# lmdu/pyfastx

Hardware: AMD Instinct MI355X
Metric: FASTA index build + 1M random 100bp subseq fetches, 3 Gbp plain FASTA per GPU (throughput of the whole step, stream resident in HBM) (higher is better)
Workload: dtype u8; 1 GPU; configs[1]: synthetic 3.0 Gbp hg38-shaped plain FASTA per GPU (200 contigs, 60-col LF, soft-masked, N runs), index build + 1000000 random 100 bp intervals (50% '-' strand); parallelism=one GPU, the whole stream resident in its HBM

## Files before the change

pyfastx_amd/csrc/fx_kernels.hpp:

```cpp
#pragma once
#include <hip/hip_runtime.h>
#include <stdint.h>

namespace fx {

constexpr int BLOCK = 256;
constexpr int UNROLL = 8;
constexpr int CHUNK = 16;
constexpr int TILE = BLOCK * CHUNK * UNROLL;

__device__ __forceinline__ uint32_t zero_bytes(uint32_t x) {
    return ~(((x & 0x7F7F7F7Fu) + 0x7F7F7F7Fu) | x | 0x7F7F7F7Fu);
}
__device__ __forceinline__ uint32_t flags4(uint32_t t) { return __builtin_amdgcn_udot4(t, 0x08040201u, 0u, false) >> 7; }
__device__ __forceinline__ uint32_t eq_mask16(const uint4 &v, uint32_t pat) {
    uint32_t lo = __builtin_amdgcn_udot4(zero_bytes(v.x ^ pat), 0x08040201u, 0u, false);
    lo = __builtin_amdgcn_udot4(zero_bytes(v.y ^ pat), 0x80402010u, lo, false);
    uint32_t hi = __builtin_amdgcn_udot4(zero_bytes(v.z ^ pat), 0x08040201u, 0u, false);
    hi = __builtin_amdgcn_udot4(zero_bytes(v.w ^ pat), 0x80402010u, hi, false);
    return (lo >> 7) | (hi << 1);
}

__device__ __forceinline__ uint4 load16(const uint8_t *__restrict__ data, int64_t p, int64_t n) {
    if (p + CHUNK <= n) return *reinterpret_cast<const uint4 *>(data + p);
// ... 327 lines not shown
                    uint32_t word = w[0];
#pragma unroll
                    for (int k = 1; k < NW; ++k) word = (j >> 2) == k ? w[k] : word;
                    uint8_t c = (uint8_t)(word >> ((j & 3) * 8));
                    if ((fl & 1) && c >= 'a' && c <= 'z') c -= 32;
                    if (fl & 4) c = lut[c];
                    const int64_t o = r - skip;
                    out[(fl & 2) ? (take - 1 - o) : o] = c;
                }
                ++r;
            }
            rank += total;
        }
        if (ok) {
            int64_t got = rank - skip;
            got = got < 0 ? 0 : (got > take ? take : got);
            if ((fl & 2) && got < take && got > 0) {
                const int64_t delta = take - got;
                for (int64_t j0 = 0; j0 < got; j0 += G) {
                    const int64_t j = j0 + sub;
                    uint8_t c = 0;
                    if (j < got) c = out[delta + j];
                    if (j < got) out[j] = c;
                }
            }
            if (sub == 0 && q.out_len) q.out_len[i] = got;
        }
    }
}

template <int G, int NP, bool COAL = false>
__global__ __launch_bounds__(BLOCK) void k_fetch_lines(const uint8_t *__restrict__ data, int64_t gbase, int64_t n_bytes, FetchQ q, FastaTab tab,
                                                      int64_t nq, int flags_all, uint8_t *__restrict__ dst, int32_t *__restrict__ list,
                                                      int *__restrict__ list_n) {
    __shared__ uint8_t lut[256];
    constexpr int CO_CAP = 2048;
    __shared__ __attribute__((aligned(16))) uint32_t s_out[COAL ? BLOCK / 64 : 1][COAL ? (CO_CAP + 32) / 4 : 1];
    constexpr int TABCAP = 512;
    __shared__ int64_t s_boff[TABCAP], s_slen[TABCAP];
    __shared__ int32_t s_llen[TABCAP], s_en[TABCAP];
    const int64_t n_seq = tab.n_seq_dev ? (*tab.n_seq_dev < tab.n_seq ? (int64_t)*tab.n_seq_dev : tab.n_seq) : tab.n_seq;
    const bool tab_lds = n_seq <= TABCAP && n_seq > 0;
    build_comp_lut(lut);
    if (tab_lds)
        for (int r = threadIdx.x; r < (int)n_seq; r += BLOCK) {
            s_boff[r] = tab.boff[r]; s_slen[r] = tab.slen[r];
            const int64_t ll = tab.llen[r];
            s_llen[r] = ll > 0x7FFFFFFFll ? 0x7FFFFFFF : (int32_t)ll;
            s_en[r] = tab.elen[r] | (tab.norm[r] << 8);
        }
    __syncthreads();
    constexpr int QPW = 64 / G;
    const int lane = lane_id(), sub = lane & (G - 1), grp = lane / G;
    const int64_t wave = ((int64_t)blockIdx.x * BLOCK + threadIdx.x) >> 6;
    const int64_t nwaves = ((int64_t)gridDim.x * BLOCK) >> 6;
    int64_t d_id = 0, d_a = 0, d_b = 0, d_off = 0;
    int d_fl = flags_all;
    auto fetch_desc = [&](int64_t i) {
        if (i >= nq) return;
        d_id = q.seq_id[i]; d_a = q.start[i]; d_b = q.stop[i];
        d_off = q.dst_off[i];
        d_fl = q.qflags ? q.qflags[i] : flags_all;
    };
    fetch_desc(wave * QPW + grp);
    for (int64_t i0 = wave * QPW; i0 < nq; i0 += nwaves * QPW) {
        const int64_t i = i0 + grp;
        const bool live = i < nq;
        const int64_t id = d_id, a = d_a, b = d_b;
// ... 339 lines not shown
```

pyfastx_amd/csrc/fx_spanscan.hpp:

```cpp
#pragma once
#include "fx_kernels.hpp"

namespace fx {

#ifndef FX_GRAN
#define FX_GRAN 4096
#endif
constexpr int GRAN = FX_GRAN;
constexpr int GR_ROWS = GRAN / (64 * CHUNK);
constexpr int SPAN_GRANS = 65536 / GRAN;
constexpr int SPAN = GRAN * SPAN_GRANS;
constexpr uint32_t SP_NONE = 0xFFFFFFFFu;

struct GranOut { uint32_t n, h, first, last, v1, c1, v2, c2, ovf; };
struct __attribute__((aligned(16))) GranPk { uint32_t nh, fl, d1, d2; };
__device__ __forceinline__ GranPk gran_pack(const GranOut &o) {
    GranPk p;
    p.nh = o.n | (o.h << 16); p.fl = (o.first & 0xFFFFu) | (o.last << 16);
    p.d1 = o.v1 | (o.c1 << 16); p.d2 = o.v2 | (o.c2 << 16) | (o.ovf << 31);
    return p;
}
__device__ __forceinline__ GranOut gran_unpack(const GranPk &p) {
    GranOut o;
    o.n = p.nh & 0xFFFFu; o.h = p.nh >> 16;
// ... 240 lines not shown
    const int lo = __shfl((int)(v & 0xFFFFFFFFll), l, 64), hi = __shfl((int)(v >> 32), l, 64);
    return ((long long)hi << 32) | (unsigned int)lo;
}
struct Tri { long long n, h, last; };
__device__ __forceinline__ Tri tri_join(const Tri &a, const Tri &b) { return Tri{a.n + b.n, a.h + b.h, a.last > b.last ? a.last : b.last}; }
__device__ __forceinline__ Tri tri_wave_incl(Tri v) {
    const int l = lane_id();
#pragma unroll
    for (int d = 1; d < 64; d <<= 1) {
        const Tri t{shfl_up64(v.n, d), shfl_up64(v.h, d), shfl_up64(v.last, d)};
        if (l >= d) v = tri_join(t, v);
    }
    return v;
}
__device__ __forceinline__ Tri tri_block_incl(Tri v, Tri *lds, Tri *total) {
    const int w = threadIdx.x >> 6, l = lane_id(), nw = (blockDim.x + 63) >> 6;
    const Tri inc = tri_wave_incl(v);
    __syncthreads();
    if (l == 63) lds[w] = inc;
    __syncthreads();
    Tri base{0, 0, -1}, tot{0, 0, -1};
    for (int i = 0; i < nw; ++i) { const Tri s = lds[i]; if (i < w) base = tri_join(base, s); tot = tri_join(tot, s); }
    *total = tot;
    return tri_join(base, inc);
}
__device__ __forceinline__ Tri gran_tri(const GranPk *__restrict__ go, int64_t g, int64_t ngran, int64_t gbase) {
    if (g >= ngran) return Tri{0, 0, -1};
    const GranOut o = gran_unpack(go[g]);
    return Tri{(long long)o.n, (long long)o.h, o.n ? gbase + g * (long long)GRAN + o.last : -1};
}

template <int MODE, int CG>
__global__ __launch_bounds__(CG) void k_gran_reduce(const uint8_t *__restrict__ data, int64_t n, int prev_byte,
                                                   int is_last, GranList hgl, GranPk *__restrict__ go,
                                                   int64_t ngran, int64_t gbase, ChunkTot *__restrict__ ct) {
    __shared__ Tri lds[CG / 64];
    if (blockIdx.x == gridDim.x - 1) {
        if (threadIdx.x < 64) {
            uint32_t L = 0;
            const uint32_t h_w = granule<false, MODE>(data, n, prev_byte, is_last, ngran - 1, go, L);
            if (MODE == 0 && h_w && threadIdx.x == 0) hgl.g[atomicAdd(hgl.count, 1u)] = (uint32_t)(ngran - 1);
        }
        __threadfence_block();
        __syncthreads();
    }
    Tri tot;
    tri_block_incl(gran_tri(go, (int64_t)blockIdx.x * CG + threadIdx.x, ngran, gbase), lds, &tot);
    if (threadIdx.x == 0) ct[blockIdx.x] = ChunkTot{tot.n, tot.h, tot.last, 0};
}

struct Tri32 { uint32_t n, h; int32_t last; };
__device__ __forceinline__ Tri32 tri32_block_incl(Tri32 v, uint32_t (*lds)[16], Tri32 *total) {
    const int w = threadIdx.x >> 6, l = lane_id(), nw = (blockDim.x + 63) >> 6;
#pragma unroll
    for (int d = 1; d < 64; d <<= 1) {
        const uint32_t a = __shfl_up(v.n, d, 64), b = __shfl_up(v.h, d, 64);
        const int32_t c = __shfl_up(v.last, d, 64);
        if (l >= d) { v.n += a; v.h += b; v.last = c > v.last ? c : v.last; }
    }
    __syncthreads();
    if (l == 63) { lds[0][w] = v.n; lds[1][w] = v.h; lds[2][w] = (uint32_t)v.last; }
    __syncthreads();
    Tri32 base{0, 0, -1}, tot{0, 0, -1};
    for (int i = 0; i < nw; ++i) {
        const uint32_t a = lds[0][i], b = lds[1][i];
        const int32_t c = (int32_t)lds[2][i];
        if (i < w) { base.n += a; base.h += b; base.last = c > base.last ? c : base.last; }
        tot.n += a; tot.h += b; tot.last = c > tot.last ? c : tot.last;
    }
    *total = tot;
    return Tri32{base.n + v.n, base.h + v.h, base.last > v.last ? base.last : v.last};
}

template <int CG>
__global__ __launch_bounds__(CG) void k_gran_prefix(const GranPk *__restrict__ go, int64_t ngran, int64_t gbase,
                                                            const ChunkTot *__restrict__ ct, Totals *__restrict__ tot,
                                                            int64_t *__restrict__ nl_prefix, int64_t *__restrict__ hdr_prefix,
                                                            int64_t *__restrict__ prevnl) {
    __shared__ Tri lds[CG / 64];
    __shared__ uint32_t lds32[3][16];
    Tri b{0, 0, -1};
    for (int64_t c = threadIdx.x; c < (int64_t)blockIdx.x; c += CG) { const ChunkTot t = ct[c]; b = tri_join(b, Tri{t.n, t.h, t.last}); }
    Tri base{0, 0, -1};
    if (blockIdx.x) tri_block_incl(b, lds, &base);
    const int64_t g = (int64_t)blockIdx.x * CG + threadIdx.x;
    Tri32 v{0, 0, -1};
    if (g < ngran) {
        const GranOut o = gran_unpack(go[g]);
        v = Tri32{o.n, o.h, o.n ? (int32_t)(threadIdx.x * GRAN + o.last) : -1};
    }
    Tri32 total;
    const Tri32 inc = tri32_block_incl(v, lds32, &total);
    const int64_t cstart = gbase + (int64_t)blockIdx.x * CG * GRAN;
    if (g < ngran) {
        nl_prefix[g] = base.n + (inc.n - v.n);
        hdr_prefix[g] = base.h + (inc.h - v.h);
        int32_t pm = __shfl_up(inc.last, 1, 64);
        if (lane_id() == 0) { pm = -1; for (int i = 0; i < (int)(threadIdx.x >> 6); ++i) { const int32_t c = (int32_t)lds32[2][i]; pm = c > pm ? c : pm; } }
        prevnl[g] = pm >= 0 ? cstart + pm : base.last;
    }
    if (blockIdx.x == gridDim.x - 1 && threadIdx.x == 0) {
        const int64_t tn = base.n + total.n, th = base.h + total.h, tl = total.last >= 0 ? cstart + total.last : base.last;
        nl_prefix[ngran] = tn; hdr_prefix[ngran] = th; prevnl[ngran] = tl;
        tot->n_nl = tn; tot->n_hdr = th; tot->last_nl = tl;
    }
}

struct ScanCtx {
    const uint8_t *data; int64_t n, gbase, ngran;
    const GranPk *go;
    const int64_t *nl_prefix, *hdr_prefix, *prevnl;
};

__device__ __forceinline__ int64_t next_nl(const ScanCtx &c, int64_t x) {
    const int64_t y = x + 1 - c.gbase;
    if (y > c.n) return -1;
    const int64_t g = y / GRAN;
    if (g < c.ngran) {
        const GranOut o = gran_unpack(c.go[g]);
        const int64_t gs = g * (int64_t)GRAN;
        if (o.n && gs + o.last >= y) {
            if (gs + o.first >= y) return c.gbase + gs + o.first;
            for (int64_t p = y & ~(int64_t)(CHUNK - 1); p < gs + GRAN; p += CHUNK) {
                const uint4 v = load16(c.data, p, c.n);
                uint32_t m = eq_mask16(v, 0x0A0A0A0Au);
                if (p < y) m &= 0xFFFFu << (y - p);
                if (m) return c.gbase + p + (__ffs(m) - 1);
                if (p + CHUNK > c.n) break;
            }
            return c.gbase + gs + o.last;
        }
    }
    const int64_t key = c.gbase + (g + 1) * (int64_t)GRAN;
    int64_t lo = g + 1, hi = c.ngran;
    if (lo >= hi || c.prevnl[c.ngran] < key) return -1;
    while (lo < hi) { const int64_t mid = (lo + hi) >> 1; if (c.prevnl[mid + 1] >= key) hi = mid; else lo = mid + 1; }
    return c.gbase + lo * (int64_t)GRAN + (c.go[lo].fl & 0xFFFFu);
// ... 281 lines not shown
            if (mism) atomicAdd(&rv.bad[r], mism);
            return;
        }
    }
    irr.g[atomicAdd(irr.count, 1u)] = (uint32_t)g;
}

__global__ __launch_bounds__(BLOCK) void k_gran_exact(ScanCtx x, RecView rv, int64_t cap, GranList irr, int is_last, int prev_byte) {
    const int lane = lane_id();
    const int64_t wave = ((int64_t)blockIdx.x * blockDim.x + threadIdx.x) >> 6;
    const int64_t nwaves = ((int64_t)gridDim.x * blockDim.x) >> 6;
    const int64_t cnt = *irr.count;
    int64_t i = wave, g = i < cnt ? irr.g[i] : 0;
    uint4 v[GR_ROWS];
    if (i < cnt) {
#pragma unroll
        for (int j = 0; j < GR_ROWS; ++j) v[j] = load16(x.data, g * (int64_t)GRAN + j * 1024 + lane * CHUNK, x.n);
    }
    for (; i < cnt; i += nwaves) {
        const int64_t gc = g, hb = x.hdr_prefix[gc];
        int64_t he = x.hdr_prefix[gc + 1];
        if (he > cap) he = cap;
        ExactMasks mk;
        exact_masks(x, v, is_last, prev_byte, gc, he > hb, mk);
        if (i + nwaves < cnt) {
            g = irr.g[i + nwaves];
#pragma unroll
            for (int j = 0; j < GR_ROWS; ++j) v[j] = load16(x.data, g * (int64_t)GRAN + j * 1024 + lane * CHUNK, x.n);
        }
        exact_rows(x, rv, cap, gc, hb, mk);
    }
}

__global__ __launch_bounds__(BLOCK) void k_fasta_finalize2(int64_t cap, FastaCols c, Totals *__restrict__ tot,
                                                          const uint8_t *__restrict__ data, int64_t n_bytes, int64_t gbase) {
    const int64_t *__restrict__ hdr = c.hoff, *__restrict__ hdr_line = c.hdr_line;
    const int64_t k = (int64_t)blockIdx.x * BLOCK + threadIdx.x;
    const int64_t n_hdr = tot->n_hdr < cap ? tot->n_hdr : cap;
    int64_t s = 0;
    if (k < n_hdr) {
        if (c.dlen[k] >= 0) {
            int64_t hn, Ln;
            if (k + 1 < n_hdr) { hn = hdr[k + 1]; Ln = hdr_line[k + 1]; }
            else               { hn = tot->last_nl + 1; Ln = tot->n_nl; }
            const int64_t nseq = Ln - hdr_line[k] - 1;
            const int64_t blen = hn - c.boff[k];
            s = blen - (int64_t)c.elen[k] * nseq;
            c.blen[k] = blen; c.slen[k] = s;
            const int norm = c.bad[k] > 1 ? 0 : 1;
            c.norm[k] = norm;
            int reg = line_regular(data, n_bytes, gbase, c.boff[k], blen, s, nseq > 0 ? c.llen[k] : 0, c.elen[k], norm);
            if (reg < 0) reg = c.bad[k] == 0;
            c.reg[k] = reg;
        } else { c.blen[k] = 0; c.slen[k] = 0; c.norm[k] = 1; c.reg[k] = 0; }
    }
    __shared__ unsigned long long blk;
    if (threadIdx.x == 0) blk = 0;
    __syncthreads();
    s = wave_sum64(s);
    if (lane_id() == 0 && s) atomicAdd(&blk, (unsigned long long)s);
    __syncthreads();
    if (threadIdx.x == 0 && blk) atomicAdd((unsigned long long *)&tot->seq_len, blk);
}

__global__ __launch_bounds__(BLOCK) void k_line_regular(const uint8_t *__restrict__ data, int64_t n_bytes, int64_t gbase, int64_t n,
                                                       const int64_t *__restrict__ boff, const int64_t *__restrict__ blen,
                                                       const int64_t *__restrict__ slen, const int64_t *__restrict__ llen,
                                                       const int32_t *__restrict__ elen, const int32_t *__restrict__ norm,
                                                       int32_t *__restrict__ reg) {
    const int64_t k = (int64_t)blockIdx.x * BLOCK + threadIdx.x;
    if (k < n) reg[k] = line_regular(data, n_bytes, gbase, boff[k], blen[k], slen[k], llen[k], elen[k], norm[k]) > 0 ? 1 : 0;
}

__device__ __forceinline__ int64_t prev_nl_wave(const ScanCtx &x, int64_t p) {
    const int64_t y = (p - x.gbase < x.n) ? p - x.gbase : x.n;
    if (y <= 0) return -1;
    const int64_t g = (y - 1) / GRAN;
    const int64_t a = g * (int64_t)GRAN + lane_id() * 64;
    unsigned long long m = 0;
#pragma unroll
    for (int i = 0; i < 4; ++i)
        if (a + i * CHUNK < y) m |= (unsigned long long)eq_mask16(load16(x.data, a + i * CHUNK, x.n), 0x0A0A0A0Au) << (16 * i);
    if (y - a < 64) m &= (y - a <= 0) ? 0ull : (~0ull >> (64 - (y - a)));
    const unsigned long long b = __ballot(m != 0);
    if (!b) return x.prevnl[g];
    const int l = 63 - __clzll(b);
    const int hi = __shfl((int)(m >> 32), l, 64), lo = __shfl((int)(m & 0xFFFFFFFFull), l, 64);
    const unsigned long long ml = ((unsigned long long)(unsigned int)hi << 32) | (unsigned int)lo;
    return x.gbase + g * (int64_t)GRAN + l * 64 + (63 - __clzll(ml));
}

constexpr int SUMM_BLOCK = 1024;
__device__ __forceinline__ DiffSet diffset_shfl_xor(const DiffSet &d, int m) {
    return DiffSet{(uint32_t)__shfl_xor((int)d.v1, m, 64), (uint32_t)__shfl_xor((int)d.c1, m, 64), (uint32_t)__shfl_xor((int)d.v2, m, 64),
                   (uint32_t)__shfl_xor((int)d.c2, m, 64), (uint32_t)__shfl_xor((int)d.ovf, m, 64)};
// ... 210 lines not shown
```

pyfastx_amd/csrc/fxgpu.hip:

```cpp
#include <hip/hip_runtime.h>
#include <zlib.h>
#include <fcntl.h>
#include <pthread.h>
#include <sched.h>
#include <sys/mman.h>
#include <sys/stat.h>
#include <unistd.h>

#include <algorithm>
#include <atomic>
#include <chrono>
#include <functional>
#include <map>
#include <memory>
#include <cstdarg>
#include <cstdio>
#include <cstdlib>
#include <cstring>
#include <mutex>
#include <string>
#include <thread>
#include <vector>

#include "../../include/fxgpu.h"
// ... 315 lines not shown
        (h)->prof.end((h)->stream);                                               \
    } while (0)
#define FX_LAUNCH_LDS(h, id, kern, grid, block, lds, ...)                         \
    do {                                                                          \
        (h)->prof.begin(id, (h)->stream);                                         \
        hipLaunchKernelGGL(kern, grid, block, lds, (h)->stream, __VA_ARGS__);     \
        (h)->prof.end((h)->stream);                                               \
    } while (0)

struct StageAsync;
static void stage_drop(fx_handle *h);
struct fx_handle {
    int device = 0;
    hipStream_t stream = nullptr;
    StageAsync *stage = nullptr;
    int stage_fd = -1;
    hipStream_t stream2 = nullptr;
    uint8_t *d_data = nullptr;
    uint8_t *d_alloc = nullptr;
    size_t blob_cap = 0;
    bool owns = false;
    int64_t n = 0;
    bool gz = false;
    int64_t base = 0;
    int prev_byte = '\n';
    bool is_last = true;
    int64_t n_nl = 0;
    bool scanned = false;
    int64_t ngran = 0;
    DevBuf<GranPk> gran;
    DevBuf<uint32_t> hdr_grans, irr_grans;
    DevBuf<ChunkTot> chunks;
    DevBuf<unsigned long long> ctl;
    Totals *pin_tot = nullptr;
    struct OneBox { int64_t off, blen, skip, take, dst_off, out_len; } *one_box = nullptr;
    uint8_t *one_out = nullptr;
    Mailbox *mb = nullptr;
    hipStream_t mb_stream = nullptr;
    unsigned long long mb_seq = 0;
    bool mb_running = false, mb_off = false;
    DevBuf<uint32_t> nm_table;
    DevBuf<int64_t> nm_off;
    uint64_t nm_mask = 0;
    int nm_kind = -1;
    DevBuf<int64_t> nl_prefix, hdr_prefix, prevnl;
    DevBuf<int64_t> hdr, fa_boff, fa_blen, fa_slen, fa_llen, fa_hdr_line;
    DevBuf<int32_t> fa_elen, fa_norm, fa_dlen, fa_name_len, fa_reg;
    DevBuf<uint32_t> fa_bad;
    int64_t n_hdr = 0, fa_seqlen = 0;
    bool fasta_built = false;
    bool build_pending = false;
    int pending_full_name = 0;
    DevBuf<uint32_t> comp_runs;
    int comp_gpw = 0;
    bool comp_runs_valid = false;
    DevBuf<int64_t> fq_name_off, fq_rlen, fq_soff, fq_qoff;
    DevBuf<int32_t> fq_name_len, fq_dlen, fq_qlen;
    DevBuf<FastqAcc> fq_acc;
    DevBuf<FqRun> fq_runs;
    DevBuf<FastqAcc> fq_acc_build;
    DevBuf<uint32_t> fq_rej;
    int64_t fq_comp_runs = 0, fq_comp_rejected = 0;
    bool fq_comp_valid = false;
    int64_t fq_comp_base[5] = {0, 0, 0, 0, 0};
    int fq_comp_minqs = 104, fq_comp_maxqs = 33;
    DevBuf<uint32_t> fq_lines;
// ... 1523 lines not shown
            unsigned char c = buf[i];
            if (!(c == ' ' || (c >= 9 && c <= 13))) { *out = c; return FX_OK; }
        }
    }
    return FX_OK;
}


static ScanCtx scan_ctx(const fx_handle *h) {
    ScanCtx x;
    x.data = h->d_data; x.n = h->n; x.gbase = h->base; x.ngran = h->ngran;
    x.go = h->gran.p; x.nl_prefix = h->nl_prefix.p; x.hdr_prefix = h->hdr_prefix.p; x.prevnl = h->prevnl.p;
    return x;
}
static FastaCols fasta_cols(fx_handle *h) {
    FastaCols c;
    c.hoff = h->hdr.p; c.boff = h->fa_boff.p; c.blen = h->fa_blen.p; c.slen = h->fa_slen.p; c.llen = h->fa_llen.p;
    c.hdr_line = h->fa_hdr_line.p; c.elen = h->fa_elen.p; c.dlen = h->fa_dlen.p; c.name_len = h->fa_name_len.p;
    c.norm = h->fa_norm.p; c.bad = h->fa_bad.p; c.reg = h->fa_reg.p;
    return c;
}
static int alloc_fasta_table(fx_handle *h, int64_t cap) {
    int rc;
    if ((rc = h->hdr.alloc(cap)) || (rc = h->fa_hdr_line.alloc(cap)) || (rc = h->fa_boff.alloc(cap)) ||
        (rc = h->fa_blen.alloc(cap)) || (rc = h->fa_slen.alloc(cap)) || (rc = h->fa_llen.alloc(cap)) ||
        (rc = h->fa_elen.alloc(cap)) || (rc = h->fa_norm.alloc(cap)) || (rc = h->fa_dlen.alloc(cap)) ||
        (rc = h->fa_name_len.alloc(cap)) || (rc = h->fa_bad.alloc(cap)) || (rc = h->fa_reg.alloc(cap)))
        return rc;
    return FX_OK;
}

static Totals *ctl_totals(fx_handle *h) { return (Totals *)h->ctl.p; }
static uint32_t *ctl_counter(fx_handle *h, int i) { return (uint32_t *)(h->ctl.p + 8 + i); }

static int comp_run_granules(int64_t ngran) {
    return ngran >= 65536 ? 4 * COMP_DEPTH : ngran >= 16384 ? 2 * COMP_DEPTH : COMP_DEPTH;
}

template <int MODE>
static int granule_pass(fx_handle *h, bool fq_lines = false, bool with_comp = false) {
    int rc;
    const int64_t nfull = h->n / GRAN, ngran = nfull + 1;
    const bool small = ngran <= (2ll << 20);
    const int64_t cg = small ? 256 : 1024, nchunks = (ngran + cg - 1) / cg;
    h->ngran = ngran;
    if ((rc = h->gran.alloc(ngran)) || (rc = h->hdr_grans.alloc(ngran)) || (MODE == 0 && (rc = h->irr_grans.alloc(ngran))) ||
        (rc = h->chunks.alloc(nchunks)) ||
        (rc = h->ctl.alloc(64)) || (rc = h->nl_prefix.alloc(ngran + 1)) || (rc = h->hdr_prefix.alloc(ngran + 1)) ||
        (rc = h->prevnl.alloc(ngran + 1)))
        return rc;
    if (!h->pin_tot) HIPCHK(hipHostMalloc((void **)&h->pin_tot, sizeof(Totals), hipHostMallocDefault));
    HIPCHK(hipMemsetAsync(h->ctl.p, 0, 64 * sizeof(unsigned long long), h->stream));
    GranList hgl{h->hdr_grans.p, ctl_counter(h, 0)};
    const int SCAN_WG = 512;
    if (nfull > 0 && MODE == 1 && fq_lines) {
        if ((rc = h->fq_lines.alloc((nfull + FQR_G - 1) / FQR_G * FQR_G * FQL_CAP))) return rc;
        if (with_comp) {
            const int64_t nruns = (nfull + FQLC_G - 1) / FQLC_G;
            if ((rc = h->fq_runs.alloc(nruns)) || (rc = h->fq_acc_build.alloc(1)) || (rc = h->fq_rej.alloc(nruns + 1))) return rc;
            static const int64_t grid_cap = [] { const char *e = getenv("FX_FQ_FUSED_GRID"); return e && atoll(e) > 0 ? atoll(e) : 6144ll; }();
            static const int force_crlf = [] { const char *e = getenv("FX_FQ_CRLF"); return e ? atoi(e) : -1; }();
            if (force_crlf >= 0 ? force_crlf != 0 : h->fq_crlf)
                FX_LAUNCH(h, K_FASTQ_LINES, k_fastq_lines_comp<true>, dim3((unsigned)std::min<int64_t>(nblocks(nruns, BLOCK / 64), grid_cap)), dim3(BLOCK), h->d_data,
                          h->n, h->prev_byte, nfull, h->gran.p, h->fq_lines.p, hgl, h->fq_runs.p, nruns);
            else
                FX_LAUNCH(h, K_FASTQ_LINES, k_fastq_lines_comp<false>, dim3((unsigned)std::min<int64_t>(nblocks(nruns, BLOCK / 64), grid_cap)), dim3(BLOCK), h->d_data,
                          h->n, h->prev_byte, nfull, h->gran.p, h->fq_lines.p, hgl, h->fq_runs.p, nruns);
        } else
        FX_LAUNCH(h, K_FASTQ_LINES, k_fastq_lines, dim3(nblocks(nfull, (BLOCK / 64) * FQL_G)), dim3(BLOCK), h->d_data, h->n, h->prev_byte, nfull,
                  h->gran.p, h->fq_lines.p, hgl);
    } else if (nfull > 0 && MODE == 0 && with_comp) {
        const int gpw = comp_run_granules(ngran);
        const int64_t runs = (ngran + gpw - 1) / gpw;
        if ((rc = h->comp_runs.alloc(runs * RUN_WORDS))) return rc;
        HIPCHK(hipMemsetAsync(h->comp_runs.p, 0, (size_t)runs * RUN_WORDS * 4, h->stream));
        FX_LAUNCH(h, K_SCAN_COMP, k_scan_comp, dim3(nblocks(runs, COMP_WPB)), dim3(COMP_WPB * 64), h->d_data, h->n, h->prev_byte,
                  (int)h->is_last, nfull, h->gran.p, hgl, gpw, h->comp_runs.p);
        h->comp_gpw = gpw;
        h->comp_runs_valid = true;
    } else if (nfull > 0)
        FX_LAUNCH(h, K_SPAN_SCAN, (k_span_scan<MODE>), dim3(nblocks((nfull + SCAN_GPW - 1) / SCAN_GPW * 64, SCAN_WG)), dim3(SCAN_WG), h->d_data, h->n,
                  h->prev_byte, (int)h->is_last, nfull, h->gran.p, hgl);
    if (small) {
        FX_LAUNCH(h, K_GRAN_REDUCE, (k_gran_reduce<MODE, 256>), dim3((unsigned)nchunks), dim3(256), h->d_data, h->n, h->prev_byte,
                  (int)h->is_last, hgl, h->gran.p, ngran, h->base, h->chunks.p);
        FX_LAUNCH(h, K_GRAN_PREFIX, (k_gran_prefix<256>), dim3((unsigned)nchunks), dim3(256), h->gran.p, ngran, h->base,
                  h->chunks.p, ctl_totals(h), h->nl_prefix.p, h->hdr_prefix.p, h->prevnl.p);
    } else {
        FX_LAUNCH(h, K_GRAN_REDUCE, (k_gran_reduce<MODE, 1024>), dim3((unsigned)nchunks), dim3(1024), h->d_data, h->n, h->prev_byte,
                  (int)h->is_last, hgl, h->gran.p, ngran, h->base, h->chunks.p);
        FX_LAUNCH(h, K_GRAN_PREFIX, (k_gran_prefix<1024>), dim3((unsigned)nchunks), dim3(1024), h->gran.p, ngran, h->base,
                  h->chunks.p, ctl_totals(h), h->nl_prefix.p, h->hdr_prefix.p, h->prevnl.p);
    }
    if (MODE == 1 && fq_lines && with_comp && nfull > 0) {
        FastqAcc init;
        memset(&init, 0, sizeof init);
        init.minqs = 104; init.maxqs = 33;
        HIPCHK(hipMemcpyAsync(h->fq_acc_build.p, &init, sizeof init, hipMemcpyHostToDevice, h->stream));
        const int64_t nruns = (nfull + FQLC_G - 1) / FQLC_G;
        HIPCHK(hipMemsetAsync(h->fq_rej.p, 0, 4, h->stream));
        FX_LAUNCH(h, K_FASTQ_COMP, k_fastq_comp_reduce, dim3((unsigned)std::min<int64_t>(nblocks(nruns, BLOCK), 1024)), dim3(BLOCK), (const FqRun *)h->fq_runs.p,
                  nruns, (const int64_t *)h->nl_prefix.p, (int64_t)0, h->d_data, h->n, nfull, h->fq_acc_build.p, h->fq_rej.p);
    }
    HIPCHK(hipGetLastError());
    return FX_OK;
}

static int enqueue_records(fx_handle *h, int full_name) {
    const ScanCtx x = scan_ctx(h);
    const int64_t cap = h->hdr.cap, ngran = h->ngran;
    const FastaCols c = fasta_cols(h);
    const RecView rv{h->fa_boff.p, h->fa_llen.p, h->fa_dlen.p, h->fa_bad.p, h->hdr.p};
    const GranList hgl{h->hdr_grans.p, ctl_counter(h, 0)}, irr{h->irr_grans.p, ctl_counter(h, 1)};
    FX_LAUNCH(h, K_HDR_REC, k_hdr_rec, dim3(2048), dim3(BLOCK), x, h->prev_byte, (int)h->is_last, full_name, hgl, c, cap);
    FX_LAUNCH(h, K_GRAN_LINES, k_gran_lines, dim3(nblocks(ngran, BLOCK)), dim3(BLOCK), x, rv, cap, irr);
    FX_LAUNCH(h, K_GRAN_EXACT, k_gran_exact, dim3(2048), dim3(BLOCK), x, rv, cap, irr, (int)h->is_last, h->prev_byte);
    FX_LAUNCH(h, K_FASTA_FINALIZE, k_fasta_finalize2, dim3(nblocks(cap, BLOCK)), dim3(BLOCK), cap, c, ctl_totals(h), h->d_data, h->n, h->base);
    HIPCHK(hipGetLastError());
    HIPCHK(hipMemcpyAsync(h->pin_tot, ctl_totals(h), sizeof(Totals), hipMemcpyDeviceToHost, h->stream));
    return FX_OK;
}

extern "C" int fx_fasta_build_begin(fx_handle *h, int full_name) {
    if (!h) return fail(FX_EINVAL, "null handle");
    int rc = use_device(h);
    if (rc) return rc;
    if (h->n <= 0) return fail(FX_EFORMAT, "empty input");
    h->scanned = false;
    h->nm_kind = -1;
    const bool with_comp = (full_name & 2) != 0;
    full_name &= 1;
    h->comp_runs_valid = h->rk_valid = false;
    if ((rc = granule_pass<0>(h, false, with_comp))) return rc;
    if (h->hdr.cap < 4096 && (rc = alloc_fasta_table(h, 4096))) return rc;
    if ((rc = enqueue_records(h, full_name))) return rc;
    h->build_pending = true;
    h->pending_full_name = full_name;
    h->fasta_built = true;
    return FX_OK;
}

static int finish_build(fx_handle *h) {
    if (!h->build_pending) return FX_OK;
    int rc = use_device(h);
    if (rc) return rc;
    Totals tot;
    for (;;) {
        HIPCHK(hipStreamSynchronize(h->stream));
        tot = *h->pin_tot;
        if (tot.n_hdr <= h->hdr.cap) break;
        if ((rc = alloc_fasta_table(h, tot.n_hdr + tot.n_hdr / 16 + 16))) return rc;
        HIPCHK(hipMemsetAsync(&ctl_totals(h)->seq_len, 0, 8, h->stream));
        HIPCHK(hipMemsetAsync(ctl_counter(h, 1), 0, 4, h->stream));
        if ((rc = enqueue_records(h, h->pending_full_name))) return rc;
    }
    h->build_pending = false;
    h->n_hdr = tot.n_hdr;
    h->n_nl = tot.n_nl;
    h->fa_seqlen = tot.seq_len;
    if (tot.n_hdr <= 0 && h->base == 0 && h->is_last) { h->fasta_built = false; return fail(FX_EFORMAT, "no FASTA header line ('>') found"); }
    return FX_OK;
}

extern "C" int fx_fasta_build_end(fx_handle *h, fx_fasta_summary *out) {
    if (!h) return fail(FX_EINVAL, "null handle");
    if (!h->fasta_built) return fail(FX_ESTATE, "fx_fasta_build_begin has not run");
    int rc = finish_build(h);
    if (rc) return rc;
    if (out) { out->n_seq = h->n_hdr; out->seq_len = h->fa_seqlen; out->n_lines = h->n_nl; out->n_bytes = h->n; }
    return FX_OK;
}

extern "C" int fx_fasta_build(fx_handle *h, int full_name, fx_fasta_summary *out) {
    int rc = fx_fasta_build_begin(h, full_name);
    if (rc) return rc;
    return fx_fasta_build_end(h, out);
}

extern "C" int fx_fasta_set_table(fx_handle *h, int64_t n, const int64_t *boff, const int64_t *blen, const int64_t *slen,
                                  const int64_t *llen, const int32_t *elen, const int32_t *norm) {
    if (!h || n < 0 || (n > 0 && (!boff || !blen || !slen || !llen || !elen || !norm))) return fail(FX_EINVAL, "bad argument");
    int rc = use_device(h);
    if (rc) return rc;
    h->rk_valid = false;
    if ((rc = alloc_fasta_table(h, std::max<int64_t>(n, 1)))) return rc;
    auto up = [&](void *d, const void *s_, size_t bytes) { return hipMemcpyAsync(d, s_, bytes, hipMemcpyHostToDevice, h->stream); };
    if (n) {
// ... 663 lines not shown
            h->pin_in_used += padded;
        }
        hipError_t e = hipMemcpyAsync(d, from, (size_t)bytes, hipMemcpyHostToDevice, h->stream);
        if (e != hipSuccess) return fail(FX_EDEVICE, "H2D: %s", hipGetErrorString(e));
        *dst = (const T *)d;
        return FX_OK;
    }
    template <class T> int scratch(int64_t n, T **dst) {
        void *d = take(n * (int64_t)sizeof(T));
        if (!d) return fail(FX_ENOMEM, "device scratch allocation failed");
        *dst = (T *)d;
        return FX_OK;
    }
};

static unsigned fetch_grid(int64_t nq) {
    static const int64_t cap = []() { const char *e = getenv("FX_FETCH_WG"); const int64_t v = e ? atoll(e) : 0; return v > 0 ? v : (int64_t)256 * 8 * 4; }();
    return (unsigned)std::max<int64_t>(1, std::min<int64_t>((nq + 3) / 4, cap));
}

static int fetch_launch(fx_handle *h, Staged &st, const FetchQ &q, bool by_id, bool longq, int64_t n, int flags, uint8_t *d_dst) {
    int rc;
    FastaTab tab;
    memset(&tab, 0, sizeof tab);
    if (h->fasta_built) {
        tab.boff = h->fa_boff.p; tab.blen = h->fa_blen.p; tab.slen = h->fa_slen.p; tab.llen = h->fa_llen.p;
        tab.elen = h->fa_elen.p; tab.norm = h->fa_reg.p; tab.n_seq = h->n_hdr;
        if (h->build_pending) { tab.n_seq_dev = (const long long *)&ctl_totals(h)->n_hdr; tab.n_seq = h->hdr.cap; }
    }
    static const int fetch_g = [] { const char *e = getenv("FX_FETCH_G"); return e ? atoi(e) : 4; }();
    static const bool lean = [] { const char *e = getenv("FX_FETCH_LEAN"); return !e || atoi(e) != 0; }();
    if (!longq && by_id && fetch_g == 4 && lean && n < 0x7FFFFFFFll) {
        int32_t *d_list = nullptr;
        int *d_cnt = nullptr;
        if ((rc = st.scratch<int32_t>(n, &d_list)) || (rc = st.scratch<int>(1, &d_cnt))) return rc;
        HIPCHK(hipMemsetAsync(d_cnt, 0, sizeof(int), h->stream));
        static const int np = [] { const char *e = getenv("FX_FETCH_NP"); return e ? atoi(e) : 1; }();
        static const bool coal = [] { const char *e = getenv("FX_FETCH_COAL"); return e && atoi(e) != 0; }();
        if (np == 1 && coal) FX_LAUNCH(h, K_FETCH, (k_fetch_lines<4, 1, true>), dim3(fetch_grid((n + 15) / 16)), dim3(BLOCK), h->d_data, h->base, h->n, q, tab, n, flags, d_dst, d_list, d_cnt);
        else if (np == 1) FX_LAUNCH(h, K_FETCH, (k_fetch_lines<4, 1>), dim3(fetch_grid((n + 15) / 16)), dim3(BLOCK), h->d_data, h->base, h->n, q, tab, n, flags, d_dst, d_list, d_cnt);
        else         FX_LAUNCH(h, K_FETCH, (k_fetch_lines<4, 2>), dim3(fetch_grid((n + 15) / 16)), dim3(BLOCK), h->d_data, h->base, h->n, q, tab, n, flags, d_dst, d_list, d_cnt);
        FX_LAUNCH(h, K_FETCH_REST, (k_fetch<true, 4, 16>), dim3(std::min(fetch_grid((n + 15) / 16), 1024u)), dim3(BLOCK), h->d_data, h->base, h->n, q, tab, n, flags,
                  d_dst, (const int32_t *)d_list, (const int *)d_cnt);
    } else if (!longq && by_id && fetch_g == 4) {
        FX_LAUNCH(h, K_FETCH, (k_fetch<true, 4, 16>), dim3(fetch_grid((n + 15) / 16)), dim3(BLOCK), h->d_data, h->base, h->n, q, tab, n, flags, d_dst);
    } else if (!longq && by_id && fetch_g == 2) {
        FX_LAUNCH(h, K_FETCH, (k_fetch<true, 2, 16>), dim3(fetch_grid((n + 31) / 32)), dim3(BLOCK), h->d_data, h->base, h->n, q, tab, n, flags, d_dst);
    } else if (!longq && by_id && fetch_g == 16) {
        FX_LAUNCH(h, K_FETCH, (k_fetch<true, 16, 16>), dim3(fetch_grid((n + 3) / 4)), dim3(BLOCK), h->d_data, h->base, h->n, q, tab, n, flags, d_dst);
    } else if (!longq) {
        const unsigned grid8 = fetch_grid((n + 7) / 8);
        if (by_id) FX_LAUNCH(h, K_FETCH, (k_fetch<true, 8, 16>), dim3(grid8), dim3(BLOCK), h->d_data, h->base, h->n, q, tab, n, flags, d_dst);
        else       FX_LAUNCH(h, K_FETCH, (k_fetch<false, 8, 16>), dim3(grid8), dim3(BLOCK), h->d_data, h->base, h->n, q, tab, n, flags, d_dst);
    } else {
        const unsigned grid = fetch_grid(n);
        if (by_id) FX_LAUNCH(h, K_FETCH, (k_fetch<true, 64, 16>), dim3(grid), dim3(BLOCK), h->d_data, h->base, h->n, q, tab, n, flags, d_dst);
        else       FX_LAUNCH(h, K_FETCH, (k_fetch<false, 64, 16>), dim3(grid), dim3(BLOCK), h->d_data, h->base, h->n, q, tab, n, flags, d_dst);
    }
    HIPCHK(hipGetLastError());
    return FX_OK;
}

static int fetch_common(fx_handle *h, int where, int64_t n, bool by_id, const int64_t *a0, const int64_t *a1,
                        const int64_t *a2, const int64_t *skip, int flags, const uint8_t *qflags, uint8_t *dst,
                        const int64_t *dst_off, int64_t *out_len, int64_t dst_bytes_hint) {
    if (!h) return fail(FX_EINVAL, "null handle");
    if (n < 0 || (n > 0 && (!a0 || !a1 || !a2 || !dst || !dst_off))) return fail(FX_EINVAL, "null query array");
    if (by_id && !h->fasta_built) return fail(FX_ESTATE, "fx_fasta_build has not run");
    if (n == 0) return FX_OK;
    int rc = use_device(h);
    if (rc) return rc;
    Staged st(h);
    FetchQ q;
    memset(&q, 0, sizeof q);
    const int64_t *host_blen = (where == FX_HOST && !by_id) ? a1 : nullptr;
    uint8_t *d_dst = dst;
// ... 4376 lines not shown
```

Measured before the change: 4874 Gbp/s.

## Fold counter resets and totals readback into kernels to drop memset/memcpy ops

Replaces several stream-ordered memsets and the device-to-host totals memcpy with in-kernel work. Counters are reset by the kernels that consume them, the fetch list counter is double-buffered so the next call's counter is zeroed by the current fetch kernel, and the finalize kernel uses a last-block ticket to write totals directly into pinned host memory. The finalize grid is also capped, with a grid-stride loop over headers. This removes small per-call API operations and launches from the critical path, at the cost of more complex state tracking (ctl_clean flag, ticket ordering) and reliance on system-scope fences for host visibility.

```diff
diff --git a/pyfastx_amd/csrc/fx_kernels.hpp b/pyfastx_amd/csrc/fx_kernels.hpp
--- a/pyfastx_amd/csrc/fx_kernels.hpp
+++ b/pyfastx_amd/csrc/fx_kernels.hpp
@@ -383,8 +383,9 @@
 template <int G, int NP, bool COAL = false>
 __global__ __launch_bounds__(BLOCK) void k_fetch_lines(const uint8_t *__restrict__ data, int64_t gbase, int64_t n_bytes, FetchQ q, FastaTab tab,
                                                       int64_t nq, int flags_all, uint8_t *__restrict__ dst, int32_t *__restrict__ list,
-                                                      int *__restrict__ list_n) {
+                                                      int *__restrict__ list_n, int *__restrict__ next_list_n) {
     __shared__ uint8_t lut[256];
+    if (blockIdx.x == 0 && threadIdx.x == 0) *next_list_n = 0;
     constexpr int CO_CAP = 2048;
     __shared__ __attribute__((aligned(16))) uint32_t s_out[COAL ? BLOCK / 64 : 1][COAL ? (CO_CAP + 32) / 4 : 1];
     constexpr int TABCAP = 512;
diff --git a/pyfastx_amd/csrc/fx_spanscan.hpp b/pyfastx_amd/csrc/fx_spanscan.hpp
--- a/pyfastx_amd/csrc/fx_spanscan.hpp
+++ b/pyfastx_amd/csrc/fx_spanscan.hpp
@@ -296,14 +296,17 @@
 
 template <int MODE, int CG>
 __global__ __launch_bounds__(CG) void k_gran_reduce(const uint8_t *__restrict__ data, int64_t n, int prev_byte,
-                                                   int is_last, GranList hgl, GranPk *__restrict__ go,
+                                                   int is_last, GranList hgl, uint32_t *__restrict__ hdr_count, GranPk *__restrict__ go,
                                                    int64_t ngran, int64_t gbase, ChunkTot *__restrict__ ct) {
     __shared__ Tri lds[CG / 64];
     if (blockIdx.x == gridDim.x - 1) {
         if (threadIdx.x < 64) {
             uint32_t L = 0;
             const uint32_t h_w = granule<false, MODE>(data, n, prev_byte, is_last, ngran - 1, go, L);
-            if (MODE == 0 && h_w && threadIdx.x == 0) hgl.g[atomicAdd(hgl.count, 1u)] = (uint32_t)(ngran - 1);
+            if (threadIdx.x == 0) {
+                if (MODE == 0 && h_w) hgl.g[atomicAdd(hgl.count, 1u)] = (uint32_t)(ngran - 1);
+                *hdr_count = atomicExch(hgl.count, 0u);
+            }
         }
         __threadfence_block();
         __syncthreads();
@@ -340,7 +343,8 @@
 __global__ __launch_bounds__(CG) void k_gran_prefix(const GranPk *__restrict__ go, int64_t ngran, int64_t gbase,
                                                             const ChunkTot *__restrict__ ct, Totals *__restrict__ tot,
                                                             int64_t *__restrict__ nl_prefix, int64_t *__restrict__ hdr_prefix,
-                                                            int64_t *__restrict__ prevnl) {
+                                                            int64_t *__restrict__ prevnl, uint32_t *__restrict__ irr_count,
+                                                            int *__restrict__ stitch_err) {
     __shared__ Tri lds[CG / 64];
     __shared__ uint32_t lds32[3][16];
     Tri b{0, 0, -1};
@@ -367,6 +371,7 @@
         const int64_t tn = base.n + total.n, th = base.h + total.h, tl = total.last >= 0 ? cstart + total.last : base.last;
         nl_prefix[ngran] = tn; hdr_prefix[ngran] = th; prevnl[ngran] = tl;
         tot->n_nl = tn; tot->n_hdr = th; tot->last_nl = tl;
+        tot->seq_len = 0; *irr_count = 0; *stitch_err = 0;
     }
 }
 
@@ -714,17 +719,20 @@
     }
 }
 
+constexpr int FINALIZE_MAX_WG = 2048;
 __global__ __launch_bounds__(BLOCK) void k_fasta_finalize2(int64_t cap, FastaCols c, Totals *__restrict__ tot,
-                                                          const uint8_t *__restrict__ data, int64_t n_bytes, int64_t gbase) {
+                                                          const uint8_t *__restrict__ data, int64_t n_bytes, int64_t gbase,
+                                                          Totals *__restrict__ host_tot, uint32_t *__restrict__ ticket) {
     const int64_t *__restrict__ hdr = c.hoff, *__restrict__ hdr_line = c.hdr_line;
-    const int64_t k = (int64_t)blockIdx.x * BLOCK + threadIdx.x;
     const int64_t n_hdr = tot->n_hdr < cap ? tot->n_hdr : cap;
-    int64_t s = 0;
-    if (k < n_hdr) {
+    const int64_t t_nl = tot->n_nl, t_hdr = tot->n_hdr, t_last = tot->last_nl;
+    int64_t sum = 0;
+    for (int64_t k = (int64_t)blockIdx.x * BLOCK + threadIdx.x; k < n_hdr; k += (int64_t)gridDim.x * BLOCK) {
+        int64_t s = 0;
         if (c.dlen[k] >= 0) {
             int64_t hn, Ln;
             if (k + 1 < n_hdr) { hn = hdr[k + 1]; Ln = hdr_line[k + 1]; }
-            else               { hn = tot->last_nl + 1; Ln = tot->n_nl; }
+            else               { hn = t_last + 1; Ln = t_nl; }
             const int64_t nseq = Ln - hdr_line[k] - 1;
             const int64_t blen = hn - c.boff[k];
             s = blen - (int64_t)c.elen[k] * nseq;
@@ -735,14 +743,24 @@
             if (reg < 0) reg = c.bad[k] == 0;
             c.reg[k] = reg;
         } else { c.blen[k] = 0; c.slen[k] = 0; c.norm[k] = 1; c.reg[k] = 0; }
+        sum += s;
     }
     __shared__ unsigned long long blk;
     if (threadIdx.x == 0) blk = 0;
     __syncthreads();
-    s = wave_sum64(s);
-    if (lane_id() == 0 && s) atomicAdd(&blk, (unsigned long long)s);
+    sum = wave_sum64(sum);
+    if (lane_id() == 0 && sum) atomicAdd(&blk, (unsigned long long)sum);
     __syncthreads();
-    if (threadIdx.x == 0 && blk) atomicAdd((unsigned long long *)&tot->seq_len, blk);
+    if (threadIdx.x == 0) {
+        if (blk) atomicAdd((unsigned long long *)&tot->seq_len, blk);
+        asm volatile("s_waitcnt vmcnt(0)" ::: "memory");
+        if (atomicAdd(ticket, 1u) == gridDim.x - 1) {
+            atomicExch(ticket, 0u);
+            const long long seq_len = (long long)atomicAdd((unsigned long long *)&tot->seq_len, 0ull);
+            host_tot->n_nl = t_nl; host_tot->n_hdr = t_hdr; host_tot->last_nl = t_last; host_tot->seq_len = seq_len;
+            __threadfence_system();
+        }
+    }
 }
 
 __global__ __launch_bounds__(BLOCK) void k_line_regular(const uint8_t *__restrict__ data, int64_t n_bytes, int64_t gbase, int64_t n,
diff --git a/pyfastx_amd/csrc/fxgpu.hip b/pyfastx_amd/csrc/fxgpu.hip
--- a/pyfastx_amd/csrc/fxgpu.hip
+++ b/pyfastx_amd/csrc/fxgpu.hip
@@ -371,6 +371,9 @@
     DevBuf<uint32_t> hdr_grans, irr_grans;
     DevBuf<ChunkTot> chunks;
     DevBuf<unsigned long long> ctl;
+    bool ctl_clean = false;
+    DevBuf<int> fetch_cnt;
+    unsigned fetch_calls = 0;
     Totals *pin_tot = nullptr;
     struct OneBox { int64_t off, blen, skip, take, dst_off, out_len; } *one_box = nullptr;
     uint8_t *one_out = nullptr;
@@ -1960,6 +1963,8 @@
 
 static Totals *ctl_totals(fx_handle *h) { return (Totals *)h->ctl.p; }
 static uint32_t *ctl_counter(fx_handle *h, int i) { return (uint32_t *)(h->ctl.p + 8 + i); }
+static uint32_t *ctl_append(fx_handle *h) { return (uint32_t *)(h->ctl.p + 10); }
+static uint32_t *ctl_ticket(fx_handle *h) { return (uint32_t *)(h->ctl.p + 11); }
 
 static int comp_run_granules(int64_t ngran) {
     return ngran >= 65536 ? 4 * COMP_DEPTH : ngran >= 16384 ? 2 * COMP_DEPTH : COMP_DEPTH;
@@ -1978,8 +1983,9 @@
         (rc = h->prevnl.alloc(ngran + 1)))
         return rc;
     if (!h->pin_tot) HIPCHK(hipHostMalloc((void **)&h->pin_tot, sizeof(Totals), hipHostMallocDefault));
-    HIPCHK(hipMemsetAsync(h->ctl.p, 0, 64 * sizeof(unsigned long long), h->stream));
-    GranList hgl{h->hdr_grans.p, ctl_counter(h, 0)};
+    if (!h->ctl_clean) HIPCHK(hipMemsetAsync(h->ctl.p, 0, 64 * sizeof(unsigned long long), h->stream));
+    h->ctl_clean = false;
+    GranList hgl{h->hdr_grans.p, ctl_append(h)};
     const int SCAN_WG = 512;
     if (nfull > 0 && MODE == 1 && fq_lines) {
         if ((rc = h->fq_lines.alloc((nfull + FQR_G - 1) / FQR_G * FQR_G * FQL_CAP))) return rc;
@@ -2011,14 +2017,14 @@
                   h->prev_byte, (int)h->is_last, nfull, h->gran.p, hgl);
     if (small) {
         FX_LAUNCH(h, K_GRAN_REDUCE, (k_gran_reduce<MODE, 256>), dim3((unsigned)nchunks), dim3(256), h->d_data, h->n, h->prev_byte,
-                  (int)h->is_last, hgl, h->gran.p, ngran, h->base, h->chunks.p);
+                  (int)h->is_last, hgl, ctl_counter(h, 0), h->gran.p, ngran, h->base, h->chunks.p);
         FX_LAUNCH(h, K_GRAN_PREFIX, (k_gran_prefix<256>), dim3((unsigned)nchunks), dim3(256), h->gran.p, ngran, h->base,
-                  h->chunks.p, ctl_totals(h), h->nl_prefix.p, h->hdr_prefix.p, h->prevnl.p);
+                  h->chunks.p, ctl_totals(h), h->nl_prefix.p, h->hdr_prefix.p, h->prevnl.p, ctl_counter(h, 1), (int *)(h->ctl.p + 60));
     } else {
         FX_LAUNCH(h, K_GRAN_REDUCE, (k_gran_reduce<MODE, 1024>), dim3((unsigned)nchunks), dim3(1024), h->d_data, h->n, h->prev_byte,
-                  (int)h->is_last, hgl, h->gran.p, ngran, h->base, h->chunks.p);
+                  (int)h->is_last, hgl, ctl_counter(h, 0), h->gran.p, ngran, h->base, h->chunks.p);
         FX_LAUNCH(h, K_GRAN_PREFIX, (k_gran_prefix<1024>), dim3((unsigned)nchunks), dim3(1024), h->gran.p, ngran, h->base,
-                  h->chunks.p, ctl_totals(h), h->nl_prefix.p, h->hdr_prefix.p, h->prevnl.p);
+                  h->chunks.p, ctl_totals(h), h->nl_prefix.p, h->hdr_prefix.p, h->prevnl.p, ctl_counter(h, 1), (int *)(h->ctl.p + 60));
     }
     if (MODE == 1 && fq_lines && with_comp && nfull > 0) {
         FastqAcc init;
@@ -2031,6 +2037,7 @@
                   nruns, (const int64_t *)h->nl_prefix.p, (int64_t)0, h->d_data, h->n, nfull, h->fq_acc_build.p, h->fq_rej.p);
     }
     HIPCHK(hipGetLastError());
+    if (MODE == 1) h->ctl_clean = true;
     return FX_OK;
 }
 
@@ -2043,9 +2050,9 @@
     FX_LAUNCH(h, K_HDR_REC, k_hdr_rec, dim3(2048), dim3(BLOCK), x, h->prev_byte, (int)h->is_last, full_name, hgl, c, cap);
     FX_LAUNCH(h, K_GRAN_LINES, k_gran_lines, dim3(nblocks(ngran, BLOCK)), dim3(BLOCK), x, rv, cap, irr);
     FX_LAUNCH(h, K_GRAN_EXACT, k_gran_exact, dim3(2048), dim3(BLOCK), x, rv, cap, irr, (int)h->is_last, h->prev_byte);
-    FX_LAUNCH(h, K_FASTA_FINALIZE, k_fasta_finalize2, dim3(nblocks(cap, BLOCK)), dim3(BLOCK), cap, c, ctl_totals(h), h->d_data, h->n, h->base);
+    FX_LAUNCH(h, K_FASTA_FINALIZE, k_fasta_finalize2, dim3(std::min<unsigned>(nblocks(cap, BLOCK), FINALIZE_MAX_WG)), dim3(BLOCK), cap, c, ctl_totals(h),
+              h->d_data, h->n, h->base, h->pin_tot, ctl_ticket(h));
     HIPCHK(hipGetLastError());
-    HIPCHK(hipMemcpyAsync(h->pin_tot, ctl_totals(h), sizeof(Totals), hipMemcpyDeviceToHost, h->stream));
     return FX_OK;
 }
 
@@ -2062,6 +2069,7 @@
     if ((rc = granule_pass<0>(h, false, with_comp))) return rc;
     if (h->hdr.cap < 4096 && (rc = alloc_fasta_table(h, 4096))) return rc;
     if ((rc = enqueue_records(h, full_name))) return rc;
+    h->ctl_clean = true;
     h->build_pending = true;
     h->pending_full_name = full_name;
     h->fasta_built = true;
@@ -2077,10 +2085,12 @@
         HIPCHK(hipStreamSynchronize(h->stream));
         tot = *h->pin_tot;
         if (tot.n_hdr <= h->hdr.cap) break;
+        h->ctl_clean = false;
         if ((rc = alloc_fasta_table(h, tot.n_hdr + tot.n_hdr / 16 + 16))) return rc;
         HIPCHK(hipMemsetAsync(&ctl_totals(h)->seq_len, 0, 8, h->stream));
         HIPCHK(hipMemsetAsync(ctl_counter(h, 1), 0, 4, h->stream));
         if ((rc = enqueue_records(h, h->pending_full_name))) return rc;
+        h->ctl_clean = true;
     }
     h->build_pending = false;
     h->n_hdr = tot.n_hdr;
@@ -2810,16 +2820,23 @@
     static const bool lean = [] { const char *e = getenv("FX_FETCH_LEAN"); return !e || atoi(e) != 0; }();
     if (!longq && by_id && fetch_g == 4 && lean && n < 0x7FFFFFFFll) {
         int32_t *d_list = nullptr;
-        int *d_cnt = nullptr;
-        if ((rc = st.scratch<int32_t>(n, &d_list)) || (rc = st.scratch<int>(1, &d_cnt))) return rc;
-        HIPCHK(hipMemsetAsync(d_cnt, 0, sizeof(int), h->stream));
+        if ((rc = st.scratch<int32_t>(n, &d_list))) return rc;
+        if (!h->fetch_cnt.p) {
+            if ((rc = h->fetch_cnt.alloc(2))) return rc;
+            const hipError_t e = hipMemsetAsync(h->fetch_cnt.p, 0, 2 * sizeof(int), h->stream);
+            if (e != hipSuccess) { h->fetch_cnt.release(); return fail(FX_EDEVICE, "fill: %s", hipGetErrorString(e)); }
+            h->fetch_calls = 0;
+        }
+        int *d_cnt = h->fetch_cnt.p + (h->fetch_calls & 1u), *d_cnt_next = h->fetch_cnt.p + (~h->fetch_calls & 1u);
+        ++h->fetch_calls;
         static const int np = [] { const char *e = getenv("FX_FETCH_NP"); return e ? atoi(e) : 1; }();
         static const bool coal = [] { const char *e = getenv("FX_FETCH_COAL"); return e && atoi(e) != 0; }();
-        if (np == 1 && coal) FX_LAUNCH(h, K_FETCH, (k_fetch_lines<4, 1, true>), dim3(fetch_grid((n + 15) / 16)), dim3(BLOCK), h->d_data, h->base, h->n, q, tab, n, flags, d_dst, d_list, d_cnt);
-        else if (np == 1) FX_LAUNCH(h, K_FETCH, (k_fetch_lines<4, 1>), dim3(fetch_grid((n + 15) / 16)), dim3(BLOCK), h->d_data, h->base, h->n, q, tab, n, flags, d_dst, d_list, d_cnt);
-        else         FX_LAUNCH(h, K_FETCH, (k_fetch_lines<4, 2>), dim3(fetch_grid((n + 15) / 16)), dim3(BLOCK), h->d_data, h->base, h->n, q, tab, n, flags, d_dst, d_list, d_cnt);
+        if (np == 1 && coal) FX_LAUNCH(h, K_FETCH, (k_fetch_lines<4, 1, true>), dim3(fetch_grid((n + 15) / 16)), dim3(BLOCK), h->d_data, h->base, h->n, q, tab, n, flags, d_dst, d_list, d_cnt, d_cnt_next);
+        else if (np == 1) FX_LAUNCH(h, K_FETCH, (k_fetch_lines<4, 1>), dim3(fetch_grid((n + 15) / 16)), dim3(BLOCK), h->d_data, h->base, h->n, q, tab, n, flags, d_dst, d_list, d_cnt, d_cnt_next);
+        else         FX_LAUNCH(h, K_FETCH, (k_fetch_lines<4, 2>), dim3(fetch_grid((n + 15) / 16)), dim3(BLOCK), h->d_data, h->base, h->n, q, tab, n, flags, d_dst, d_list, d_cnt, d_cnt_next);
         FX_LAUNCH(h, K_FETCH_REST, (k_fetch<true, 4, 16>), dim3(std::min(fetch_grid((n + 15) / 16), 1024u)), dim3(BLOCK), h->d_data, h->base, h->n, q, tab, n, flags,
                   d_dst, (const int32_t *)d_list, (const int *)d_cnt);
+        if (hipPeekAtLastError() != hipSuccess) h->fetch_cnt.release();
     } else if (!longq && by_id && fetch_g == 4) {
         FX_LAUNCH(h, K_FETCH, (k_fetch<true, 4, 16>), dim3(fetch_grid((n + 15) / 16)), dim3(BLOCK), h->d_data, h->base, h->n, q, tab, n, flags, d_dst);
     } else if (!longq && by_id && fetch_g == 2) {
```

New measurement: 4915 Gbp/s (median of 4 runs). Within noise of the previous version (+0.8%).
